# stephane-caron/pink

Measured on AMD Instinct MI355X. Metric: ik_qp_solves_per_s, higher is better.
Workload: dtype f64

## Files before the change

### pink_amd/csrc/ik_common.h

```cpp
#pragma once

#include <cmath>
#include <cstdint>
#include <type_traits>

#ifndef PINKHIP_GROUP_LARGE
#define PINKHIP_GROUP_LARGE 8
#endif
#ifndef PINKHIP_GROUP_SMALL
#define PINKHIP_GROUP_SMALL 4
#endif

#if defined(PINKHIP_TRACE) && !defined(__HIP_DEVICE_COMPILE__)
#include <cstdio>
#define PINKHIP_TRACEF(cond, ...)        \
  do {                                   \
    if (cond) std::printf(__VA_ARGS__);  \
  } while (0)
#else
#define PINKHIP_TRACEF(cond, ...)
#endif

namespace pinkhip {

template <int NV>
constexpr int group_size() {
  return NV >= 24 ? PINKHIP_GROUP_LARGE : PINKHIP_GROUP_SMALL;
}

template <int I, int N, class F>
__device__ __forceinline__ void static_for(F &&f) {
  if constexpr (I < N) {
    f(std::integral_constant<int, I>{});
    static_for<I + 1, N>(f);
  }
}
template <int W, int N, int BIT, class F>
__device__ __forceinline__ double transpose_reduce(F v) {
  const int lane = lane_id();
  if constexpr ((1 << BIT) >= W) {
    static_assert(N == 1, "N <= W values fold to one per lane");
    return v(std::integral_constant<int, 0>{});
  } else {
    constexpr int H = (N + 1) / 2;
    double nx[H];
    const bool up = ((lane >> BIT) & 1) != 0;
    static_for<0, H>([&](auto M) {
      constexpr int m = decltype(M)::value;
      const double a = v(std::integral_constant<int, 2 * m>{});
      double b = 0.0;
      if constexpr (2 * m + 1 < N) b = v(std::integral_constant<int, 2 * m + 1>{});
      nx[m] = (up ? b : a) + lane_shfl(up ? a : b, lane ^ (1 << BIT));
    });
    return transpose_reduce<W, H, BIT + 1>([&](auto K) { return nx[decltype(K)::value]; });
  }
}

typedef double TabVec16 __attribute__((vector_size(128)));
typedef double TabVec8 __attribute__((vector_size(64)));
template <bool HALF>
struct TabVecSel {
  typedef TabVec16 type;
};
template <>
struct TabVecSel<true> {
  typedef TabVec8 type;
};
template <int NT>
struct TabRegs {
  static constexpr int NVEC = (NT + 15) / 16;
  static_assert(NVEC >= 1 && NVEC <= 4, "at most 64 tableau columns");
  static constexpr bool kHalfLast = NT - 16 * (NVEC - 1) <= 8;
  template <int K>
  using Vec = typename TabVecSel<(K == NVEC - 1) && kHalfLast>::type;
  Vec<0> v0;
  Vec<1> v1;
  Vec<2> v2;
  Vec<3> v3;
  template <int K>
  __device__ __forceinline__ Vec<K> tuple() const {
    if constexpr (K == 0) return v0;
    else if constexpr (K == 1) return v1;
    else if constexpr (K == 2) return v2;
    else return v3;
  }
  template <int J>
  __device__ __forceinline__ double get() const {
    static_assert(J >= 0 && J < NT, "tableau column");
    const Vec<J / 16> t = tuple<J / 16>();
    return t[J % 16];
  }
  template <int J>
  __device__ __forceinline__ void set(double x) {
    static_assert(J >= 0 && J < NT, "tableau column");
    Vec<J / 16> t = tuple<J / 16>();
    t[J % 16] = x;
    if constexpr (J / 16 == 0) v0 = t;
    else if constexpr (J / 16 == 1) v1 = t;
    else if constexpr (J / 16 == 2) v2 = t;
    else v3 = t;
  }
  __device__ __forceinline__ void clear() {
    v0 = Vec<0>{};
    v1 = Vec<1>{};
    v2 = Vec<2>{};
    v3 = Vec<3>{};
  }
  __device__ __forceinline__ double at_uniform(int p) const {
    const int hi = p >> 4;
    const int lo = opaque_uniform(p & 15);
    const int lo8 = kHalfLast ? opaque_uniform(p & 7) : lo;
    const Vec<0> t0 = v0;
    double r = t0[NVEC == 1 ? lo8 : lo];
    if constexpr (NVEC > 1) {
      const Vec<1> t1 = v1;
      const double r1 = t1[NVEC == 2 ? lo8 : lo];
      r = (hi == 1) ? r1 : r;
    }
    if constexpr (NVEC > 2) {
      const Vec<2> t2 = v2;
      const double r2 = t2[NVEC == 3 ? lo8 : lo];
      r = (hi == 2) ? r2 : r;
    }
    if constexpr (NVEC > 3) {
      const Vec<3> t3 = v3;
      const double r3 = t3[lo8];
      r = (hi == 3) ? r3 : r;
    }
    return r;
  }
  template <int W>
  __device__ __forceinline__ double at_group_uniform(int p) const {
    constexpr int G = kWave / W;
    static_assert(G == 1 || G == 2, "one or two reads per wave");
    const int p0 = bcast_i(p, 0);
    double c = at_uniform(p0 < 0 ? 0 : p0);
    if constexpr (G == 2) {
      const int p1 = bcast_i(p, W);
      const double c1 = at_uniform(p1 < 0 ? 0 : p1);
      c = (lane_id() >= W) ? c1 : c;
    }
    return (p >= 0) ? c : 0.0;
  }
};

struct alignas(16) Pair {
  double a, b;
};

constexpr int STATUS_OPTIMAL = 0;
constexpr int STATUS_MAX_ITER = 1;
constexpr int STATUS_INFEASIBLE = 2;
constexpr int STATUS_NOT_PD = 3;
constexpr int STATUS_BREAKDOWN = 4;
constexpr int STATUS_ROUTED = 5;
constexpr int PATH_TABLEAU = 0, PATH_HANDOVER = 1, PATH_ROUTED = 2, PATH_GI = 3;
constexpr int kPathShift = 24;

struct KernelArgs {
  long long B;
  int nv, Kd, K, md;
  int n_eq;
  int n_dtasks;
  int n_barriers;
  int cost_batched;
  int max_iter;
  int lds_pitch;
  int rank_deficient;
  int n_free_lead;
  double damping, dt;
  double out_scale;
  const double *J, *e, *cost, *lb, *ub, *Gd, *hd, *c_extra;
  const double *row_gain;
  const double *row_lm;
  const int *dtask_col0;
  const int *dtask_row0;
  const int *dtask_k;
  const int *barrier_rows;
  const double *barrier_safe_gain;
  double *dq;
  int *status;
  int *iters;
  double *H_out, *c_out;
  const uint8_t *active_in;
  uint8_t *active_out;
};


}
// ... 1 lines not shown
```

### pink_amd/csrc/ik_stack_rows.h

```cpp
#pragma once

#include "ik_common.h"

namespace pinkhip {

struct HbmTerms {
  static constexpr bool kOnTheFly = false;
  double lb = 0.0, ub = 0.0, x = 0.0;
  int status = 0;
  __device__ __forceinline__ void frame_rows(int, double (&)[6]) const {}
  __device__ __forceinline__ double error(int) const { return 0.0; }
  __device__ __forceinline__ double diag_error(int) const { return 0.0; }
  __device__ __forceinline__ double dense_col(int) const { return 0.0; }
  __device__ __forceinline__ double dense_h(int) const { return 0.0; }
};

struct NoMid {
  __device__ __forceinline__ void operator()() const {}
};
template <int NX>
struct StackFront {
  double m[NX > 0 ? NX : 1] = {};
  double hxx[NX > 0 ? NX * (NX + 1) / 2 : 1] = {};
  double cx[NX > 0 ? NX : 1] = {};
};
template <int NV, int W, int RCMAX, class Src, int DEPTH = 1, int NX = 0, int NM, class Mid = NoMid>
__device__ __forceinline__ void stack_rows_bcast(const KernelArgs &a, long long b, Src *terms, bool in, int li,
                                                 double (&M)[NM], double &ci, double &mu_l, Mid mid = Mid(), StackFront<NX> *front = nullptr) {
  static_assert(NX >= 0 && NX <= 2 && (NX == 0 || !Src::kOnTheFly), "at most two front columns, from HBM");
  static_assert(NM >= NV && W >= 16, "row-group kernels only");
  using BcT = Bcast<W>;
  const int nv = a.nv, Kd = a.Kd, K = a.K;
  const double *Jb = a.J + b * (long long)Kd * nv;
  const double *eb = a.e + b * (long long)K;
  const double *costb = a.cost_batched ? a.cost + b * (long long)K : a.cost;
  constexpr int RC = Src::kOnTheFly ? 6 : (RCMAX < 8 ? RCMAX : 8);
  constexpr int NB = Src::kOnTheFly ? 2 : DEPTH + 1;
  static_assert(RC <= 16, "weight rows are broadcast from the first row of 16 lanes");
  struct Chunk {
    double r[RC];
    double pw, pe, pg, pl;
    double px[NX > 0 ? NX : 1];
  };
  Chunk buf[NB];
  auto request = [&](Chunk &dst, int r0) {
    const int rc = (Kd - r0 < RC) ? Kd - r0 : RC;
    if constexpr (Src::kOnTheFly) {
      double six[6];
      terms->frame_rows(r0 / 6, six);
#pragma unroll
      for (int kk = 0; kk < RC; ++kk) dst.r[kk] = (in && kk < rc) ? six[kk] : 0.0;
    } else {
#pragma unroll
      for (int kk = 0; kk < RC; ++kk) dst.r[kk] = (in && kk < rc) ? Jb[(long long)(r0 + kk) * nv + li] : 0.0;
    }
    dst.pw = dst.pe = dst.pg = dst.pl = 0.0;
    if constexpr (NX > 0) {
#pragma unroll
      for (int x = 0; x < NX; ++x) dst.px[x] = (li < rc) ? Jb[(long long)(r0 + li) * nv - NX + x] : 0.0;
    }
    if (li < rc) {
      const int k = r0 + li;
      dst.pw = costb[k];
      if constexpr (Src::kOnTheFly) dst.pe = terms->error(k);
      else dst.pe = eb[k];
      dst.pg = a.row_gain[k];
      dst.pl = a.row_lm[k];
    }
  };
  if (Kd > 0) {
#pragma unroll
    for (int d = 0; d < NB - 1; ++d)
      if (d * RC < Kd) request(buf[d], d * RC);
  }
  mid();
  for (int r0 = 0; r0 < Kd; r0 += RC) {
    const int rc = (Kd - r0 < RC) ? Kd - r0 : RC;
    if (r0 + (NB - 1) * RC < Kd) request(buf[NB - 1], r0 + (NB - 1) * RC);
    const Chunk &cur = buf[0];
    const double wa = (li < rc) ? cur.pw * cur.pw : 0.0;
    const double gw = (li < rc) ? cur.pg * wa * cur.pe : 0.0;
    if (li < rc) mu_l += cur.pl * (cur.pg * cur.pg) * wa * cur.pe * cur.pe;
    const BcT wab = bcast_prepare<W>(wa), gwb = bcast_prepare<W>(gw);
    BcT pxb[NX > 0 ? NX : 1];
    if constexpr (NX > 0) {
      front->hxx[0] = fma(wa * cur.px[0], cur.px[0], front->hxx[0]);
      front->cx[0] = fma(gw, cur.px[0], front->cx[0]);
      if constexpr (NX == 2) {
        front->hxx[1] = fma(wa * cur.px[0], cur.px[1], front->hxx[1]);
        front->hxx[2] = fma(wa * cur.px[1], cur.px[1], front->hxx[2]);
        front->cx[1] = fma(gw, cur.px[1], front->cx[1]);
      }
#pragma unroll
      for (int x = 0; x < NX; ++x) pxb[x] = bcast_prepare<W>(cur.px[x]);
    }
    static_for<0, RC>([&](auto Kc) {
      constexpr int kk = decltype(Kc)::value;
      if (kk < rc) {
        const double aa = fma_bcast<W, kk>(0.0, wab, cur.r[kk]);
        ci = fma_bcast<W, kk>(ci, gwb, cur.r[kk]);
        const BcT rowb = bcast_prepare<W>(cur.r[kk]);
        static_for<0, NV>([&](auto Jc) {
          constexpr int j = decltype(Jc)::value;
          M[j] = fma_bcast<W, j>(M[j], rowb, aa);
        });
        if constexpr (NX > 0) {
#pragma unroll
          for (int x = 0; x < NX; ++x) front->m[x] = fma_bcast<W, kk>(front->m[x], pxb[x], aa);
        }
      }
    });
#pragma unroll
    for (int d = 0; d + 1 < NB; ++d) buf[d] = buf[d + 1];
  }
}

template <class Src>
__device__ __forceinline__ double stack_diag_tasks(const KernelArgs &a, long long b, Src *terms, int li, double &ci,
                                                   double &mu_l) {
  const double *eb = a.e + b * (long long)a.K;
  const double *costb = a.cost_batched ? a.cost + b * (long long)a.K : a.cost;
  double dadd = 0.0;
  for (int t = 0; t < a.n_dtasks; ++t) {
    const int off = li - a.dtask_col0[t];
    if (off >= 0 && off < a.dtask_k[t]) {
      const int r = a.dtask_row0[t] + off;
      const double w = costb[r], gn = a.row_gain[r], l = a.row_lm[r];
      double ev;
      if constexpr (Src::kOnTheFly) ev = terms->diag_error(r);
      else ev = eb[r];
      const double wa = w * w;
      dadd += wa;
      ci += gn * wa * ev;
      mu_l += l * (gn * gn) * wa * ev * ev;
    }
  }
  return dadd;
}

}
```

### pink_amd/csrc/ik_sweep.h

```cpp
#pragma once

#include "ik_common.h"
#include "ik_kernels_packed.h"
#include "ik_stack_rows.h"

#ifdef PINKHIP_SECTION_CLOCK
#ifndef PINKHIP_TICK
static __device__ unsigned long long pinkhip_clock[16];
#define PINKHIP_TICK(k)                                                        \
  do {                                                                         \
    if (clock_on) {                                                            \
      const unsigned long long now_ = __builtin_readcyclecounter();            \
      if (lane == 0) atomicAdd(&pinkhip_clock[k], now_ - clock_prev);          \
      clock_prev = __builtin_readcyclecounter();                               \
    }                                                                          \
  } while (0)
#endif
#else
#ifndef PINKHIP_TICK
#define PINKHIP_TICK(k)
#endif
#endif

#ifndef PINKHIP_SWEEP_COLUMN_CHAINS
#define PINKHIP_SWEEP_COLUMN_CHAINS(NT) 2
#endif

#ifndef PINKHIP_SWEEP_CERT_TOL
#define PINKHIP_SWEEP_CERT_TOL 1e-12
#endif
#ifndef PINKHIP_STACK_DEPTH
#define PINKHIP_STACK_DEPTH 1
#endif
#ifndef PINKHIP_STACK_DEPTH_WIDE
#define PINKHIP_STACK_DEPTH_WIDE 2
#endif
#ifndef PINKHIP_SWEEP_INDEXED_COLUMN
#define PINKHIP_SWEEP_INDEXED_COLUMN 1
#endif
#ifndef PINKHIP_SWEEP_ROUTE_COND
#define PINKHIP_SWEEP_ROUTE_COND 1e8
#endif
#ifndef PINKHIP_SWEEP_PPM
#define PINKHIP_SWEEP_PPM 1
#endif
#ifndef PINKHIP_SWEEP_PPM_CRASH
#define PINKHIP_SWEEP_PPM_CRASH 1
#endif
#ifndef PINKHIP_ROLLOUT_PPM_DENSE
#define PINKHIP_ROLLOUT_PPM_DENSE 0
#endif
#ifndef PINKHIP_ROLLOUT_PPM_VIRTUAL
#define PINKHIP_ROLLOUT_PPM_VIRTUAL 0
#endif
#ifndef PINKHIP_SWEEP_PPM_DENSE
#define PINKHIP_SWEEP_PPM_DENSE 1
#endif
#ifdef PINKHIP_SWEEP_DEBUG_WHY
#define PINKHIP_WHY(k) why = (k) + 10 * status_before
#else
#define PINKHIP_WHY(k)
#endif
#ifndef PINKHIP_SWEEP_PPM_MIN_CURV
#define PINKHIP_SWEEP_PPM_MIN_CURV 1e-5
#endif
#ifndef PINKHIP_SWEEP_PPM_MURTY_AFTER
#define PINKHIP_SWEEP_PPM_MURTY_AFTER(nv) (4 * (nv) + 20)
#endif

namespace pinkhip {

template <int NV, int MD, int W>
struct SweepLds {
  static __host__ __device__ constexpr int tri(int i) { return i * (i + 1) / 2; }
  static constexpr int oC = (NV * (NV + 1) / 2 + 1) & ~1;
  static constexpr int GP = W + 2;
  static constexpr int oG = oC + W;
  static constexpr int oR = oG + MD * GP;
  static constexpr int stride = oR + W;
};

template <int NVT, int MD, int W, class Src = HbmTerms, bool WARM = false>
__device__ __forceinline__ int ik_sweep_instance(const KernelArgs &a, long long block, Src *terms = nullptr) {
  constexpr int NE = NVT > W ? NVT - W : 0;
  constexpr int NV = NVT - NE;
  static_assert(NE == 0 || (NE <= 2 && MD == 0 && !Src::kOnTheFly), "front coordinates are eliminated in the box-only stack + solve kernel");
  constexpr int NT = NV + MD;
  static_assert((W == 16 || W == 32 || W == 64) && NT <= W && NV % 2 == 0 && MD >= 0, "group of whole rows of 16 lanes");
  constexpr bool DENSE = MD > 0;
  constexpr bool PPM = !DENSE && PINKHIP_SWEEP_PPM;
  constexpr bool PPMD = DENSE && PINKHIP_SWEEP_PPM && PINKHIP_SWEEP_PPM_DENSE && (!Src::kOnTheFly || PINKHIP_ROLLOUT_PPM_DENSE);
  constexpr bool PPX = PPM || PPMD;
  static_assert(!WARM || PPM, "a warm start is a start of the principal pivoting of the box-only instantiations");
  constexpr int G = kWave / W;
  constexpr double INF = INFINITY;
  constexpr double BIG = 1e300;
  using BcT = Bcast<W>;

  const int lane = lane_id();
  const int g = lane / W, li = lane & (W - 1);
  const int nvs = a.nv;
  const int nv = nvs - NE;
  const int md = DENSE ? a.md : 0, n_eq = DENSE ? a.n_eq : 0;
#ifdef PINKHIP_SECTION_CLOCK
  const bool clock_on = (block & 63) == 0;
  unsigned long long clock_prev = __builtin_readcyclecounter();
#endif
  long long b = block * G + g;
  const bool valid = b < a.B;
  if (!valid) b = a.B - 1;

  const bool in = li < nv;
  const int dr = li - NV;
  const bool dlane = DENSE && dr >= 0 && dr < md;

  double T[NT];
#pragma unroll
  for (int j = 0; j < NT; ++j) T[j] = 0.0;
  double ci = 0.0, mu_l = 0.0, dadd = 0.0;
  double ci_d = 0.0, mu_d = 0.0, lbv = -INF, ubv = INF, hv = 0.0, ginv = 1.0;
  double front_dadd[NE > 0 ? NE : 1] = {}, front_c[NE > 0 ? NE : 1] = {};
  bool front_free = true;
  auto others = [&]() {
    if (in) {
      if constexpr (!Src::kOnTheFly) {
        lbv = a.lb[b * (long long)nvs + NE + li];
        ubv = a.ub[b * (long long)nvs + NE + li];
      }
      dadd = stack_diag_tasks<Src>(a, b, terms, NE + li, ci_d, mu_d);
      if (a.c_extra) ci_d += a.c_extra[b * (long long)nvs + NE + li];
    }
    if constexpr (NE > 0) {
#pragma unroll
      for (int x = 0; x < NE; ++x) {
        double mu_x = 0.0;
        front_dadd[x] = stack_diag_tasks<Src>(a, b, terms, x, front_c[x], mu_x);
        if (a.c_extra) front_c[x] += a.c_extra[b * (long long)nvs + x];
        if (li == x) mu_d += mu_x;
        front_free = front_free && a.lb[b * (long long)nvs + x] == -INF && a.ub[b * (long long)nvs + x] == INF;
      }
    }
    if constexpr (DENSE && !Src::kOnTheFly) {
      if (md > 0) {
        const double *Gb = a.Gd + b * (long long)md * nv;
        static_for<0, MD>([&](auto Dc) {
          constexpr int d = decltype(Dc)::value;
          T[NV + d] = (in && d < md) ? Gb[(long long)d * nv + li] : 0.0;
        });
        if (dlane) hv = a.hd[b * (long long)md + dr];
      }
    }
  };
  StackFront<NE> front;
  if constexpr (NE > 0) {
    KernelArgs af = a;
    af.J = a.J + NE;
    stack_rows_bcast<NV, W, 8, Src, PINKHIP_STACK_DEPTH, NE>(af, b, terms, in, li, T, ci, mu_l, others, &front);
  } else {
    stack_rows_bcast<NV, W, 8, Src, (NT > 34 ? PINKHIP_STACK_DEPTH_WIDE : PINKHIP_STACK_DEPTH)>(a, b, terms, in, li, T, ci, mu_l, others);
  }
  ci += ci_d;
  mu_l += mu_d;
  double diag = a.damping + group_sum<W>(mu_l);

  if constexpr (DENSE) {
    if (md > 0) {
      const double *Gb = Src::kOnTheFly ? nullptr : a.Gd + b * (long long)md * nv;
      if constexpr (Src::kOnTheFly) {
        static_for<0, MD>([&](auto Dc) {
          constexpr int d = decltype(Dc)::value;
          T[NV + d] = (in && d < md) ? terms->dense_col(d) : 0.0;
        });
      }
      if constexpr (Src::kOnTheFly) {
        static_for<0, MD>([&](auto Dc) {
          constexpr int d = decltype(Dc)::value;
          if (d < md) {
            const BcT gb = bcast_prepare<W>(T[NV + d]);
            static_for<0, NV>([&](auto Jc) {
              constexpr int j = decltype(Jc)::value;
              const double v = value_bcast<W, j>(gb);
              if (dr == d) T[j] = v;
            });
          }
        });
      }
      if (dlane) {
        double n2 = 0.0;
        if constexpr (!Src::kOnTheFly) {
          const double *gr = Gb + (long long)dr * nv;
#pragma unroll
          for (int j = 0; j < NV; ++j) T[j] = (j < nv) ? gr[j] : 0.0;
        } else {
          hv = terms->dense_h(dr);
        }
#pragma unroll
        for (int j = 0; j < NV; ++j) n2 += T[j] * T[j];
        ginv = (n2 > 0.0) ? 1.0 / sqrt(n2) : 1.0;
      }
      for (int t = 0; t < a.n_barriers; ++t) {
        const double r = a.barrier_safe_gain[t];
        if (r > 1e-6) {
          const int r0 = a.barrier_rows[t], r1 = a.barrier_rows[t + 1];
          double s = 0.0;
          static_for<0, MD>([&](auto Dc) {
            constexpr int d = decltype(Dc)::value;
            if (in && d >= r0 && d < r1) s += T[NV + d] * T[NV + d];
          });
          s = group_sum<W>(s);
          diag += r / (s * a.dt * a.dt);
        }
      }
    }
  }
  const double diag_u = diag;
  diag += dadd;
  double hii = 1.0;
#pragma unroll
  for (int j = 0; j < NV; ++j)
    if (j == li) {
      T[j] += in ? diag : 1.0;
      hii = T[j];
    }
  using SL = SweepLds<NV, MD, W>;
  double *sm = shared_base() + (long long)g * (a.lds_pitch ? a.lds_pitch : SL::stride);
  bool front_bad = false;
  if constexpr (NE > 0) {
    double h00 = group_sum<W>(front.hxx[0]) + diag_u + front_dadd[0];
    double c0 = group_sum<W>(front.cx[0]) + front_c[0];
    double h01 = 0.0, h11 = 1.0, c1 = 0.0;
    if constexpr (NE == 2) {
      h01 = group_sum<W>(front.hxx[1]);
      h11 = group_sum<W>(front.hxx[2]) + diag_u + front_dadd[1];
      c1 = group_sum<W>(front.cx[1]) + front_c[1];
    }
    const double m0 = in ? front.m[0] : 0.0;
    double m1 = (NE == 2 && in) ? front.m[NE - 1] : 0.0;
    front_bad = !(h00 > 0.0);
    const double r0 = fast_rcp(h00);
    {
      const BcT hb = bcast_prepare<W>(m0);
      const double f = -m0 * r0;
      static_for<0, NV>([&](auto Jc) {
        constexpr int j = decltype(Jc)::value;
        T[j] = fma_bcast<W, j>(T[j], hb, f);
      });
      ci = fma(f, c0, ci);
      hii = fma(f, m0, hii);
      if constexpr (NE == 2) {
        m1 = fma(f, h01, m1);
        h11 = fma(-h01 * r0, h01, h11);
        c1 = fma(-h01 * r0, c0, c1);
      }
    }
    double r1 = 0.0;
    if constexpr (NE == 2) {
      front_bad = front_bad || !(h11 > 0.0);
      r1 = fast_rcp(h11);
      const BcT hb = bcast_prepare<W>(m1);
      const double f = -m1 * r1;
      static_for<0, NV>([&](auto Jc) {
        constexpr int j = decltype(Jc)::value;
        T[j] = fma_bcast<W, j>(T[j], hb, f);
      });
      ci = fma(f, c1, ci);
      hii = fma(f, m1, hii);
    }
    wave_sync();
    sm[SL::stride + li] = m0;
    sm[SL::stride + W + li] = m1;
    if (li == 0) {
      double *fs = sm + SL::stride + 2 * W;
      fs[0] = c0, fs[1] = r0, fs[2] = h01, fs[3] = c1, fs[4] = r1;
    }
  }
  wave_sync();
  if (li < NV) {
#pragma unroll
    for (int j = 0; j < NV; ++j)
      if (j <= li) sm[SL::tri(li) + j] = T[j];
  }
  sm[SL::oC + li] = ci;
  if constexpr (DENSE) {
    static_for<0, MD>([&](auto Dc) {
      constexpr int d = decltype(Dc)::value;
      sm[SL::oG + d * SL::GP + li] = (li < NV) ? T[NV + d] : 0.0;
    });
  }
  PINKHIP_TICK(0);

  int status = STATUS_OPTIMAL;
  int why = 0, status_before = 0;
  if constexpr (NE > 0) {
    if (!front_free) status = STATUS_ROUTED;
    else if (front_bad) status = STATUS_NOT_PD;
  }
  double pmin = INF;
  int state = 0;
  if constexpr (Src::kOnTheFly) {
    lbv = in ? terms->lb : -INF;
    ubv = in ? terms->ub : INF;
  }
  constexpr bool GUESS = (PPX && PINKHIP_SWEEP_PPM_CRASH && !Src::kOnTheFly) || WARM;
  if constexpr (GUESS) {
    if (group_first_lane<W>(in && !(hii > 0.0)) < W) status = STATUS_NOT_PD;
    if constexpr (WARM) {
      const uint8_t *hint = a.active_in;
      if (hint) {
        if (in) {
          const int v = hint[b * (long long)nvs + NE + li];
          state = (v == 1 && lbv > -INF) ? 1 : ((v == 2 && ubv < INF) ? 2 : 0);
        }
      } else if constexpr (!Src::kOnTheFly) {
        const double xd = -ci * approx_rcp(hii);
        if (in) state = (xd < lbv) ? 1 : ((xd > ubv) ? 2 : 0);
      }
    } else {
      const double xd = -ci * approx_rcp(hii);
      if (in) state = (xd < lbv) ? 1 : ((xd > ubv) ? 2 : 0);
    }
    const unsigned long long fm = wave_ballot(li < NV && state == 0 && in);
    using FreeMask = typename std::conditional<W == 64, unsigned long long, unsigned>::type;
    FreeMask gfree = static_cast<FreeMask>(fm);
    if constexpr (W == 32) gfree = (lane >= 32) ? static_cast<unsigned>(fm >> 32) : static_cast<unsigned>(fm);
    else if constexpr (W == 16) gfree = static_cast<unsigned>(fm >> (lane & 48)) & 0xFFFFu;
    static_for<0, NV>([&](auto Kc) {
      constexpr int k = decltype(Kc)::value;
      {
        const bool want = ((gfree >> k) & 1) != 0;
        if (lanes_on(want)) {
          BcT xb = bcast_prepare<W>(T[k]);
          const double p = value_bcast<W, k>(xb);
          pmin = min_raw(pmin, want ? p : INF);
          const double rp = fast_rcp(p);
          const double t = T[k] * rp;
          double nt = (li == k) ? rp - 1.0 : -t;
          if (!want) nt = 0.0;
          double tk = (li == k) ? -rp : t;
#if defined(__HIP_DEVICE_COMPILE__)
          asm volatile("" : "+v"(nt), "+v"(xb.r[0]), "+v"(tk));
#endif
          static_for<0, NT>([&](auto Jc) {
            constexpr int j = decltype(Jc)::value;
            if constexpr (j != k) T[j] = fma_bcast<W, j>(T[j], xb, nt);
          });
          if (want) T[k] = tk;
        }
      }
    });
  }
  if constexpr (!GUESS) {
    static_for<0, NV>([&](auto Kc) {
      constexpr int k = decltype(Kc)::value;
      if (k < nv) {
        const BcT xb = bcast_prepare<W>(T[k]);
        const double p = value_bcast<W, k>(xb);
        pmin = min_raw(pmin, p);
        const double rp = fast_rcp(p);
        const double t = T[k] * rp;
        const double nt = (li == k) ? rp - 1.0 : -t;
        static_for<0, NT>([&](auto Jc) {
          constexpr int j = decltype(Jc)::value;
          if constexpr (j != k) T[j] = fma_bcast<W, j>(T[j], xb, nt);
        });
        T[k] = (li == k) ? -rp : t;
      }
    });
  }
  if (!(pmin > 0.0)) status = STATUS_NOT_PD;
  PINKHIP_TICK(1);
  double tdiag = 0.0;
#pragma unroll
  for (int j = 0; j < NT; ++j)
    if (j == li) tdiag = T[j];

  double x = 0.0, u = 0.0;
  {
    double vstart = in ? ci : 0.0;
    if constexpr (PPX) {
      if (state != 0) vstart = -((state == 1) ? lbv : ubv);
    }
    const BcT cb = bcast_prepare<W>(vstart);
    double r0 = 0.0, r1 = 0.0;
    static_for<0, NV>([&](auto Jc) {
      constexpr int j = decltype(Jc)::value;
      if constexpr (j % 2 == 0) r0 = fma_bcast<W, j>(r0, cb, T[j]);
      else r1 = fma_bcast<W, j>(r1, cb, T[j]);
    });
    x = in ? r0 + r1 : 0.0;
    if (dlane) u = hv + (r0 + r1);
    if constexpr (PPX) {
      if (state != 0) x -= ci;
    }
    if constexpr (PPMD) {
      if (dlane) x = u;
    }
  }
  double zd0 = -tdiag;
  if constexpr (PPMD) {
    const double hmax = -group_min<W>(in ? -hii : 0.0);
    zd0 = (li < NV) ? approx_rcp(hii) : approx_rcp(ginv * ginv * hmax);
  }
  {
    const double hii0 = (li < NV && in) ? sm[SL::tri(li < NV ? li : 0) + (li < NV ? li : 0)] : 0.0;
    const double kest = -group_min<W>((PPX && state != 0) ? -hii0 * approx_rcp(tdiag) : hii0 * tdiag);
    PINKHIP_TRACEF(li == 0, "[sweep g%d] kest %.3e\n", g, kest);
    if (status == STATUS_OPTIMAL && !(kest <= PINKHIP_SWEEP_ROUTE_COND)) status = STATUS_ROUTED;
  }
  PINKHIP_TICK(2);

  const KernelArgs *late = &a;
  if constexpr (!Src::kOnTheFly) late = kernarg_reload<KernelArgs>(a);
  const double tol = 1e-13 * (nv > 8 ? nv * 0.125 : 1.0);
  const double thr_lo = -tol * (1.0 + fabs(lbv)), thr_up = -tol * (1.0 + fabs(ubv));
  const double thr_d = -tol * (1.0 + fabs(hv) * ginv);
  const int max_iter = late->max_iter > 0 ? late->max_iter : 20 * (nv + md) + 50;
  const bool empty_box_somewhere = wave_any(in && ubv - lbv < (thr_lo > thr_up ? thr_lo : thr_up));
  double phi = 0.0, xfree = 1.0;
  int it = 0, eq_next = 0, src = 0, kind = 0;
  double uplus = 0.0;
  double blo = lbv, bhi = ubv, tlo = thr_lo, thi = thr_up;
  double thr_row = 0.0;
  if constexpr (PPMD) {
    thr_row = thr_d * fast_rcp(ginv);
    if (li >= NV) {
      blo = dlane ? 0.0 : -INF;
      bhi = INF;
      tlo = (dlane && dr >= n_eq) ? thr_row : -INF;
      thi = 0.0;
    }
  }
  if constexpr (PPX) {
    if (state != 0) {
      blo = (state == 1) ? -INF : 0.0;
      bhi = (state == 1) ? 0.0 : INF;
      tlo = 0.0;
      thi = 0.0;
    }
    if (empty_box_somewhere) {
      const bool empty = group_first_lane<W>(in && ubv - lbv < (thr_lo > thr_up ? thr_lo : thr_up)) < W;
      if (empty && status == STATUS_OPTIMAL) status = STATUS_INFEASIBLE;
    }
  }
  bool at_point = false;
  bool running = (status == STATUS_OPTIMAL);
  bool need_sel = true;
  bool refined = (status == STATUS_ROUTED);
  int nref = 0;
  double dprev = 0.0;

  auto krow_times = [&](double v) -> double {
    const BcT vb = bcast_prepare<W>(v);
    const int base = (li < NV) ? SL::tri(li) : SL::oG + (dlane ? dr : 0) * SL::GP;
    double h0 = 0.0, h1 = 0.0;
    static_for<0, NV>([&](auto Jc) {
      constexpr int j = decltype(Jc)::value;
      const int ad = (li < NV && j > li) ? SL::tri(j) + li : base + j;
      const double hv_ = sm[ad];
      if constexpr (j % 2 == 0) h0 = fma_bcast<W, j>(h0, vb, hv_);
      else h1 = fma_bcast<W, j>(h1, vb, hv_);
    });
    return h0 + h1;
  };
  auto residual = [&](bool &fails) -> double {
    const double kx = krow_times(in ? x : 0.0);
    const double ci_ = in ? sm[SL::oC + li] : 0.0;
    double grad = in ? kx + ci_ : 0.0;
    bool arow = false;
    if constexpr (DENSE) {
      if (md > 0) {
        arow = dlane && state == 1;
        const BcT lamb = bcast_prepare<W>(arow ? u : 0.0);
        double gl = 0.0;
        static_for<0, MD>([&](auto Dc) {
          constexpr int d = decltype(Dc)::value;
          gl = fma_bcast<W, NV + d>(gl, lamb, sm[SL::oG + d * SL::GP + li]);
        });
        if (in) grad += gl;
      }
    }
    const double hii = in ? sm[SL::tri(li < NV ? li : 0) + (li < NV ? li : 0)] : 0.0;
    const double gsc = group_min<W>(-hii) * group_min<W>(in ? -fabs(x) : 0.0) - group_min<W>(-fabs(ci_));
    const double gtol = PINKHIP_SWEEP_CERT_TOL * gsc;
    fails = false;
    if (in) {
      if (state == 0) fails = !(fabs(grad) <= gtol && x - lbv >= 10.0 * thr_lo && ubv - x >= 10.0 * thr_up);
      else fails = (state == 1) ? !(grad >= -gtol) : !(grad <= gtol);
    }
#if defined(PINKHIP_SWEEP_DEBUG_WHY) && defined(__HIP_DEVICE_COMPILE__)
    if (fails) printf("[cert blk %lld g%d li%d it%d nref%d] state %d x %.17g lb %.17g ub %.17g grad %.3e gtol %.3e thr %.3e %.3e\n", block, g, li, it, nref, state, x,
                      lbv, ubv, grad, gtol, thr_lo, thr_up);
#endif
    double r = (in && state == 0) ? grad : 0.0;
    if constexpr (DENSE) {
      if (dlane) {
        const double slack = (hv - kx) * ginv;
        if (arow) {
          r = kx - hv;
          fails = !(fabs(slack) <= -10.0 * thr_d) || (dr >= n_eq && !(u >= -gtol * ginv));
        } else if (state == 0 && dr >= n_eq) {
          fails = !(slack >= 10.0 * thr_d);
        }
      }
    }
    return r;
  };

#ifndef PINKHIP_SWEEP_LDS_COLUMN
#define PINKHIP_SWEEP_LDS_COLUMN 0
#endif
  double sdiag_run = tdiag;
  double *rowbuf = sm + SL::oR;
  constexpr bool IDX = PINKHIP_SWEEP_INDEXED_COLUMN && !PINKHIP_SWEEP_LDS_COLUMN && W >= 32;
  TabRegs<IDX ? NT : 1> R;
  R.clear();
  if constexpr (IDX) {
    static_for<0, NT>([&](auto Jc) {
      constexpr int j = decltype(Jc)::value;
      R.template set<j>(T[j]);
    });
  }
  auto tget = [&](auto Jc) -> double {
    constexpr int j = decltype(Jc)::value;
    if constexpr (IDX) return R.template get<j>();
    else return T[j];
  };
  auto tset = [&](auto Jc, double v) {
    constexpr int j = decltype(Jc)::value;
    if constexpr (IDX) R.template set<j>(v);
    else T[j] = v;
  };
  auto column_of = [&](int p) -> double {
    if constexpr (IDX) {
      return R.template at_group_uniform<W>(p);
    } else if constexpr (PINKHIP_SWEEP_LDS_COLUMN) {
      if (li == p) {
        Pair *dst = reinterpret_cast<Pair *>(__builtin_assume_aligned(rowbuf, 16));
#pragma unroll
        for (int j = 0; j + 1 < NT; j += 2) dst[j >> 1] = Pair{T[j], T[j + 1]};
        if constexpr (NT % 2) rowbuf[NT - 1] = T[NT - 1];
      }
      wave_sync();
      const double c = rowbuf[li < NT ? li : 0];
      wave_sync();
      return (p >= 0 && li < NT) ? c : 0.0;
    } else {
      const BcT eb = bcast_indicator<W>(p);
      constexpr int NC = PINKHIP_SWEEP_COLUMN_CHAINS(NT);
      double c[NC] = {};
      static_for<0, NT>([&](auto Jc) {
        constexpr int j = decltype(Jc)::value;
        c[j % NC] = fma_bcast<W, j>(c[j % NC], eb, tget(Jc));
      });
      if constexpr (NC == 4) return (c[0] + c[1]) + (c[2] + c[3]);
      else return c[0] + c[1];
    }
  };

  auto pivot_on = [&](int pi, double col, double pvt, double rp, double sg) {
    double t = col * rp;
    double cp = col;
    if (li == pi) {
      t = 1.0 - sg * rp;
      cp = pvt - sg;
    }
    const BcT xb = bcast_prepare<W>(cp);
    const double nt = -t;
    static_for<0, NT>([&](auto Jc) {
      constexpr int j = decltype(Jc)::value;
      tset(Jc, fma_bcast<W, j>(tget(Jc), xb, nt));
    });
    sdiag_run = fma(cp, nt, sdiag_run);
    tdiag = (li == pi) ? -rp : tdiag - t * col;
  };

  bool ppm_mode = PPX;
  bool restoring = false;
  const bool cand_lane = in || (DENSE && dlane && dr >= n_eq);
  const bool eq_lane = DENSE && dlane && dr < n_eq;

  for (;;) {
    double viol = 0.0;
    int nb_src = 0;
    bool iseq = false;
    if constexpr (PPX) {
      if (wave_any(running && ppm_mode)) {
        const bool sel = running && ppm_mode;
        const double slo = x - blo, sup = bhi - x;
        bool ok_lane = in, nonbasic = state != 0;
        if constexpr (DENSE) {
          nonbasic = (li < NV) ? (state != 0) : (state == 0);
          ok_lane = cand_lane && (!restoring || ((li < NV) ? (state != 0) : (state == 1)));
        }
        const bool vlo = ok_lane && slo < tlo, vup = ok_lane && sup < thi;
        viol = vlo ? slo : sup;
        if constexpr (DENSE) {
          if (eq_lane) viol = slo;
        }
        const float zf = fabsf(static_cast<float>(tdiag));
        const float wz = (zf > 1e-30f) ? approx_rcpf(zf) : 1e30f;
        const float fv = static_cast<float>(viol);
        float key = -(fv * fv) * wz;
        if (it > PINKHIP_SWEEP_PPM_MURTY_AFTER(nv + md)) key = static_cast<float>(li - 64);
        const float best32 = group_min32<W>((vlo || vup) ? key32_packf(key, li | (vlo ? 0 : 64) | (nonbasic ? 128 : 0)) : 3.0e38f);
        bool conv = false;
        if (sel) {
          if (DENSE && !restoring && eq_next < n_eq) {
            src = NV + eq_next;
            kind = 0;
            nb_src = 1;
            iseq = true;
// ... 205 lines not shown
              if (state != 0) {
                x = ((state == 1) ? lbv : ubv) + nu;
                state = 0;
                blo = lbv;
                bhi = ubv;
                tlo = thr_lo;
                thi = thr_up;
              } else {
                x = -nu;
                state = kind + 1;
                blo = kind ? 0.0 : -INF;
                bhi = kind ? INF : 0.0;
                tlo = 0.0;
                thi = 0.0;
              }
            } else if (state == 0) {
              x = nu;
              state = 1;
              tlo = 0.0;
              if (dr < n_eq) blo = -INF;
            } else {
              x = -nu;
              state = 0;
              tlo = thr_row;
            }
          }
          if constexpr (DENSE) {
            if (iseq) ++eq_next;
          }
        }
        PINKHIP_TICK(5);
        PINKHIP_TICK(6);
      }
    }
    if constexpr (!PPM) {
    if (!PPMD || wave_any(act && !ppm_mode)) {
    const bool actG = act && !ppm_mode;
    double cand = (kind == 0 ? lbv : ubv) - x;
    if constexpr (DENSE) cand = (li < NV) ? cand : -u;
    const double num = group_bcast<W>(cand, src);
    double pv = group_bcast<W>(tdiag, src);
    bool lin_dep = false;
    if constexpr (DENSE) {
      const double z0 = group_bcast<W>(zd0, src);
      const bool little = actG && !(-pv * 1e6 > z0);
      if (wave_any(little)) {
        const double w = (in && state == 0) ? col : 0.0;
        const double hw = krow_times(w);
        const double curv = group_sum<W>((li < NV) ? w * hw : 0.0);
        if (little) pv = -curv;
      }
      lin_dep = !(-pv * 1e12 > z0);
      PINKHIP_TRACEF(li == 0 && actG, "[sweep g%d it%d] enter src %d kind %d num %.3e pv %.3e z0 %.3e little %d lin_dep %d\n", g, it, src, kind,
                     num, pv, z0, (int)little, (int)lin_dep);
    }
    PINKHIP_TICK(4);
    const double rpv = fast_rcp(pv);
    const double sgn = (num >= 0.0) ? 1.0 : -1.0;
    const double full = lin_dep ? BIG : -fabs(num) * rpv;
    const double rate = phi * col * sgn;
    const bool blocking = actG && rate > 0.0;
    const double ratio = blocking ? max_raw(u, 0.0) * fast_rcp1(rate) : BIG;
    const double k1 = group_min<W>(ratio);
    const int kd = group_first_lane<W>(blocking && ratio == k1) & (W - 1);
    const double tstep = (k1 < full) ? k1 : full;
    const bool stuck = !(tstep < BIG);
    double hs = 0.0;
    if constexpr (DENSE) {
      if (wave_any(actG && stuck)) hs = group_bcast<W>((li < NV) ? (kind == 0 ? lbv : ubv) : hv, src);
    }
    if (actG && stuck) {
      const bool tiny = DENSE && fabs(num) <= 1e-9 * (1.0 + fabs(hs));
      PINKHIP_TRACEF(li == 0, "[sweep g%d it%d] stuck: src %d kind %d num %.3e hs %.3e pv %.3e lin_dep %d k1 %.3e full %.3e tiny %d\n",
                     g, it, src, kind, num, hs, pv, (int)lin_dep, k1, full, (int)tiny);
      if (kind == 3 && tiny) {
        ++eq_next;
        need_sel = true;
      } else if (tiny) {
        if (li == src) {
          if (li >= NV) hv -= u, u = 0.0;
          else if (kind == 0) lbv = x;
          else ubv = x;
        }
        need_sel = true;
      } else {
        status = STATUS_INFEASIBLE;
        running = false;
      }
    }
    const bool act2 = actG && running && !stuck;
    const bool do_add = act2 && !(k1 < full);
    const bool do_drop = act2 && !do_add;
    {
      const double nu = act2 ? sgn * tstep : 0.0;
      const double d = col * nu;
      x = fma(-xfree, d, x);
      u = fma((DENSE && li >= NV) ? -1.0 : -phi, d, u);
      if constexpr (DENSE) uplus += (kind == 3) ? nu : fabs(nu);
      else uplus += fabs(nu);
    }
    PINKHIP_TICK(5);
    if (do_add) {
      pi = src;
      pvt = pv;
      rp = rpv;
      if (li == src) {
        if (li < NV) {
          state = kind + 1;
          x = (kind == 0) ? lbv : ubv;
          phi = (kind == 0) ? -1.0 : 1.0;
        } else {
          state = 1;
          phi = (DENSE && dr >= n_eq) ? 1.0 : 0.0;
        }
        xfree = 0.0;
        u = uplus;
      }
      if (DENSE && kind == 3) ++eq_next;
      need_sel = true;
    }
    if (wave_any(do_drop)) {
      const double ck = column_of(do_drop ? kd : -1);
      const double pk = group_bcast<W>(tdiag, kd);
      if (do_drop) {
        col = (li == kd) ? tdiag : ck;
        pi = kd;
        pvt = pk;
        rp = fast_rcp(pk);
        if (li == kd) {
          state = 0;
          u = 0.0;
          phi = 0.0;
          xfree = 1.0;
        }
      }
    }
    PINKHIP_TICK(6);
    if (!ppm_mode) sg = ((!DENSE || pi < NV) == do_add) ? -1.0 : 1.0;
    }
    }
    pivot_on(pi, col, pvt, rp, sg);
    PINKHIP_TICK(7);
  }
  PINKHIP_TICK(8);
  if constexpr (Src::kOnTheFly) {
    terms->x = in ? x : 0.0;
    terms->status = status;
  }
  {
    int ln = lane;
#if defined(__HIP_DEVICE_COMPILE__)
    asm volatile("" : "+v"(ln));
#endif
    const long long bw = block * G + ln / W;
    double xe[NE > 0 ? NE : 1] = {};
    if constexpr (NE > 0) {
      const double *fs = sm + SL::stride + 2 * W;
      const double xr = in ? x : 0.0;
      if constexpr (NE == 2) xe[1] = -(fs[3] + group_sum<W>(sm[SL::stride + W + li] * xr)) * fs[4];
      xe[0] = -(fs[0] + group_sum<W>(sm[SL::stride + li] * xr) + ((NE == 2) ? fs[2] * xe[NE - 1] : 0.0)) * fs[1];
    }
    if (bw < late->B) {
      if (in) late->dq[bw * (long long)nvs + NE + li] = x * late->out_scale;
      if constexpr (NE > 0) {
        if (li < NE) late->dq[bw * (long long)nvs + li] = ((li == 0) ? xe[0] : xe[NE - 1]) * late->out_scale;
      }
      if (li == 0) {
        late->status[bw] = status;
        if (late->iters) late->iters[bw] = it + 1000 * why;
      }
      if constexpr (WARM) {
        uint8_t *const aout = late->active_out;
        if (aout) {
          if (in) aout[bw * (long long)nvs + NE + li] = static_cast<uint8_t>(status == STATUS_OPTIMAL ? state : 0);
          if constexpr (NE > 0) {
            if (li < NE) aout[bw * (long long)nvs + li] = 0;
          }
        }
      }
    }
  }
  PINKHIP_TRACEF(li == 0, "[sweep g%d] exit status %d it %d nref %d\n", g, status, it, nref);
  return status;
}

template <int NV, int MD, int W>
__host__ __device__ constexpr int sweep_kernel_lds_doubles(int md) {
  return SweepLds<NV, MD, W>::stride > LdsP<NV>::stride(MD > 0 ? md : 0) ? SweepLds<NV, MD, W>::stride : LdsP<NV>::stride(MD > 0 ? md : 0);
}

template <int NV, int MD, int W, bool WARM = false>
__device__ __forceinline__ void ik_solve_sweep_body(const KernelArgs &a, long long block) {
  const int st = ik_sweep_instance<NV, MD, W, HbmTerms, WARM>(a, block);
#ifndef PINKHIP_SWEEP_NO_HANDOVER
#ifdef PINKHIP_SWEEP_FORCE_HANDOVER
  const bool over = true;
#else
  const bool over = st == STATUS_BREAKDOWN || st == STATUS_ROUTED;
#endif
  if (wave_any(over)) {
    wave_sync();
    const KernelArgs *again = kernarg_reload<KernelArgs>(a);
    long long blk = block;
#if defined(__HIP_DEVICE_COMPILE__)
    asm volatile("" : "+s"(blk));
#endif
    if constexpr (NV > W) {
      constexpr int G = kWave / W;
      const int path = st == STATUS_ROUTED ? PATH_ROUTED : PATH_HANDOVER;
      static_for<0, G>([&](auto Gc) {
        constexpr int gg = decltype(Gc)::value;
        const bool og = bcast_i(over ? 1 : 0, gg * W) != 0;
        const int pg = bcast_i(path, gg * W);
        if (og && blk * G + gg < again->B) {
          wave_sync();
          ik_packed_instance<NV, kWave, false, HbmTerms, WARM>(*again, blk * G + gg, static_cast<HbmTerms *>(nullptr), true, pg);
        }
      });
    } else {
      ik_packed_instance<NV, W, (MD > 0), HbmTerms, WARM>(*again, blk, static_cast<HbmTerms *>(nullptr), over, st == STATUS_ROUTED ? PATH_ROUTED : PATH_HANDOVER);
    }
  }
#endif
}

template <int NV, int MD, int W>
__global__ void __launch_bounds__(kWave) PINKHIP_OCCUPANCY_SWEEP3(NV, MD, W) ik_solve_sweep_kernel(KernelArgs a) {
  ik_solve_sweep_body<NV, MD, W>(a, block_id());
}

template <int NV, int MD, int W>
__global__ void __launch_bounds__(kWave) PINKHIP_OCCUPANCY_SWEEP3(NV, MD, W) ik_solve_sweep_warm_kernel(KernelArgs a) {
  ik_solve_sweep_body<NV, MD, W, true>(a, block_id());
}

}
```

Baseline: 181.2 million.

## Use wave-uniform base pointers and track tableau diagonal in registers

```diff
diff --git a/pink_amd/csrc/ik_common.h b/pink_amd/csrc/ik_common.h
--- a/pink_amd/csrc/ik_common.h
+++ b/pink_amd/csrc/ik_common.h
@@ -35,6 +35,26 @@
     static_for<I + 1, N>(f);
   }
 }
+template <int W, int J>
+__device__ __forceinline__ double add_in_lane(double t, double d) {
+  static_assert((W == 16 || W == 32 || W == 64) && J >= 0 && J < W, "lane of a group of whole rows of 16 lanes");
+#if defined(__HIP_DEVICE_COMPILE__)
+  constexpr unsigned long long one = 1ull << J;
+  constexpr unsigned long long m = W == 64 ? one : W == 32 ? one | (one << 32) : one | (one << 16) | (one << 32) | (one << 48);
+  unsigned slo, shi;
+  asm("s_mov_b32 %1, exec_lo\n\ts_mov_b32 %2, exec_hi\n\t"
+      "s_and_b32 exec_lo, %1, %4\n\ts_and_b32 exec_hi, %2, %5\n\t"
+      "v_add_f64 %0, %0, %3\n\t"
+      "s_mov_b32 exec_lo, %1\n\ts_mov_b32 exec_hi, %2"
+      : "+v"(t), "=&s"(slo), "=&s"(shi)
+      : "v"(d), "n"(static_cast<int>(m & 0xFFFFFFFFull)), "n"(static_cast<int>(m >> 32))
+      : "scc");
+  return t;
+#else
+  return ((lane_id() & (W - 1)) == J) ? t + d : t;
+#endif
+}
+
 template <int W, int N, int BIT, class F>
 __device__ __forceinline__ double transpose_reduce(F v) {
   const int lane = lane_id();
diff --git a/pink_amd/csrc/ik_stack_rows.h b/pink_amd/csrc/ik_stack_rows.h
--- a/pink_amd/csrc/ik_stack_rows.h
+++ b/pink_amd/csrc/ik_stack_rows.h
@@ -24,16 +24,28 @@
   double hxx[NX > 0 ? NX * (NX + 1) / 2 : 1] = {};
   double cx[NX > 0 ? NX : 1] = {};
 };
-template <int NV, int W, int RCMAX, class Src, int DEPTH = 1, int NX = 0, int NM, class Mid = NoMid>
+struct WaveSplit {
+  long long first = 0;
+  unsigned rel = 0;
+};
+#ifndef PINKHIP_WAVE_SPLIT
+#define PINKHIP_WAVE_SPLIT(Src) (!Src::kOnTheFly)
+#endif
+template <int NV, int W, int RCMAX, class Src, int DEPTH = 1, int NX = 0, bool DIAG = false, int NM, class Mid = NoMid>
 __device__ __forceinline__ void stack_rows_bcast(const KernelArgs &a, long long b, Src *terms, bool in, int li,
-                                                 double (&M)[NM], double &ci, double &mu_l, Mid mid = Mid(), StackFront<NX> *front = nullptr) {
+                                                 double (&M)[NM], double &ci, double &mu_l, Mid mid = Mid(), StackFront<NX> *front = nullptr,
+                                                 double *hdiag = nullptr, WaveSplit ws = WaveSplit()) {
   static_assert(NX >= 0 && NX <= 2 && (NX == 0 || !Src::kOnTheFly), "at most two front columns, from HBM");
   static_assert(NM >= NV && W >= 16, "row-group kernels only");
   using BcT = Bcast<W>;
   const int nv = a.nv, Kd = a.Kd, K = a.K;
-  const double *Jb = a.J + b * (long long)Kd * nv;
-  const double *eb = a.e + b * (long long)K;
-  const double *costb = a.cost_batched ? a.cost + b * (long long)K : a.cost;
+  constexpr bool SPLIT = DIAG && PINKHIP_WAVE_SPLIT(Src);
+  const double *Jb = a.J + (SPLIT ? ws.first : b) * (long long)Kd * nv;
+  const double *eb = a.e + (SPLIT ? ws.first : b) * (long long)K;
+  const double *costb = a.cost_batched ? a.cost + (SPLIT ? ws.first : b) * (long long)K : a.cost;
+  const unsigned voJ = SPLIT ? ws.rel * static_cast<unsigned>(Kd * nv) + li : 0u;
+  const unsigned voE = SPLIT ? ws.rel * static_cast<unsigned>(K) + li : 0u;
+  const unsigned voC = (SPLIT && a.cost_batched) ? voE : static_cast<unsigned>(li);
   constexpr int RC = Src::kOnTheFly ? 6 : (RCMAX < 8 ? RCMAX : 8);
   constexpr int NB = Src::kOnTheFly ? 2 : DEPTH + 1;
   static_assert(RC <= 16, "weight rows are broadcast from the first row of 16 lanes");
@@ -52,20 +64,34 @@
       for (int kk = 0; kk < RC; ++kk) dst.r[kk] = (in && kk < rc) ? six[kk] : 0.0;
     } else {
 #pragma unroll
-      for (int kk = 0; kk < RC; ++kk) dst.r[kk] = (in && kk < rc) ? Jb[(long long)(r0 + kk) * nv + li] : 0.0;
+      for (int kk = 0; kk < RC; ++kk) {
+        if constexpr (SPLIT) dst.r[kk] = (in && kk < rc) ? (Jb + (long long)(r0 + kk) * nv)[voJ] : 0.0;
+        else dst.r[kk] = (in && kk < rc) ? Jb[(long long)(r0 + kk) * nv + li] : 0.0;
+      }
     }
     dst.pw = dst.pe = dst.pg = dst.pl = 0.0;
     if constexpr (NX > 0) {
 #pragma unroll
-      for (int x = 0; x < NX; ++x) dst.px[x] = (li < rc) ? Jb[(long long)(r0 + li) * nv - NX + x] : 0.0;
+      for (int x = 0; x < NX; ++x) {
+        if constexpr (SPLIT) dst.px[x] = (li < rc) ? (Jb + ((long long)r0 * nv - NX + x))[voJ - li + static_cast<unsigned>(li * nv)] : 0.0;
+        else dst.px[x] = (li < rc) ? Jb[(long long)(r0 + li) * nv - NX + x] : 0.0;
+      }
     }
     if (li < rc) {
       const int k = r0 + li;
-      dst.pw = costb[k];
-      if constexpr (Src::kOnTheFly) dst.pe = terms->error(k);
-      else dst.pe = eb[k];
-      dst.pg = a.row_gain[k];
-      dst.pl = a.row_lm[k];
+      if constexpr (SPLIT) {
+        dst.pw = (costb + r0)[voC];
+        if constexpr (Src::kOnTheFly) dst.pe = terms->error(k);
+        else dst.pe = (eb + r0)[voE];
+        dst.pg = (a.row_gain + r0)[static_cast<unsigned>(li)];
+        dst.pl = (a.row_lm + r0)[static_cast<unsigned>(li)];
+      } else {
+        dst.pw = costb[k];
+        if constexpr (Src::kOnTheFly) dst.pe = terms->error(k);
+        else dst.pe = eb[k];
+        dst.pg = a.row_gain[k];
+        dst.pl = a.row_lm[k];
+      }
     }
   };
   if (Kd > 0) {
@@ -99,6 +125,7 @@
       if (kk < rc) {
         const double aa = fma_bcast<W, kk>(0.0, wab, cur.r[kk]);
         ci = fma_bcast<W, kk>(ci, gwb, cur.r[kk]);
+        if constexpr (DIAG) *hdiag = fma(cur.r[kk], aa, *hdiag);
         const BcT rowb = bcast_prepare<W>(cur.r[kk]);
         static_for<0, NV>([&](auto Jc) {
           constexpr int j = decltype(Jc)::value;
@@ -138,4 +165,29 @@
   return dadd;
 }
 
+template <class Src>
+__device__ __forceinline__ double stack_diag_tasks(const KernelArgs &a, WaveSplit ws, Src *terms, int li, double &ci,
+                                                   double &mu_l) {
+  const double *eb = a.e + ws.first * (long long)a.K;
+  const double *costb = a.cost_batched ? a.cost + ws.first * (long long)a.K : a.cost;
+  const unsigned vo = ws.rel * static_cast<unsigned>(a.K);
+  const unsigned voc = a.cost_batched ? vo : 0u;
+  double dadd = 0.0;
+  for (int t = 0; t < a.n_dtasks; ++t) {
+    const int off = li - a.dtask_col0[t];
+    if (off >= 0 && off < a.dtask_k[t]) {
+      const int r = a.dtask_row0[t] + off;
+      const double w = costb[voc + static_cast<unsigned>(r)], gn = a.row_gain[r], l = a.row_lm[r];
+      double ev;
+      if constexpr (Src::kOnTheFly) ev = terms->diag_error(r);
+      else ev = eb[vo + static_cast<unsigned>(r)];
+      const double wa = w * w;
+      dadd += wa;
+      ci += gn * wa * ev;
+      mu_l += l * (gn * gn) * wa * ev * ev;
+    }
+  }
+  return dadd;
 }
+
+}
diff --git a/pink_amd/csrc/ik_sweep.h b/pink_amd/csrc/ik_sweep.h
--- a/pink_amd/csrc/ik_sweep.h
+++ b/pink_amd/csrc/ik_sweep.h
@@ -68,6 +68,13 @@
 #define PINKHIP_SWEEP_PPM_MURTY_AFTER(nv) (4 * (nv) + 20)
 #endif
 
+#ifndef PINKHIP_SWEEP_DIAG_REGISTER
+#define PINKHIP_SWEEP_DIAG_REGISTER(Src) (!Src::kOnTheFly)
+#endif
+#ifndef PINKHIP_SWEEP_LATE_ADDRESSES
+#define PINKHIP_SWEEP_LATE_ADDRESSES(Src) (!Src::kOnTheFly)
+#endif
+
 namespace pinkhip {
 
 template <int NV, int MD, int W>
@@ -88,6 +95,7 @@
   constexpr int NT = NV + MD;
   static_assert((W == 16 || W == 32 || W == 64) && NT <= W && NV % 2 == 0 && MD >= 0, "group of whole rows of 16 lanes");
   constexpr bool DENSE = MD > 0;
+  constexpr bool DREG = PINKHIP_SWEEP_DIAG_REGISTER(Src);
   constexpr bool PPM = !DENSE && PINKHIP_SWEEP_PPM;
   constexpr bool PPMD = DENSE && PINKHIP_SWEEP_PPM && PINKHIP_SWEEP_PPM_DENSE && (!Src::kOnTheFly || PINKHIP_ROLLOUT_PPM_DENSE);
   constexpr bool PPX = PPM || PPMD;
@@ -109,6 +117,10 @@
   long long b = block * G + g;
   const bool valid = b < a.B;
   if (!valid) b = a.B - 1;
+  WaveSplit ws;
+  ws.first = (block * G < a.B - 1) ? block * G : a.B - 1;
+  ws.rel = static_cast<unsigned>(b - ws.first);
+  const unsigned vo = ws.rel * static_cast<unsigned>(nvs) + li;
 
   const bool in = li < nv;
   const int dr = li - NV;
@@ -124,11 +136,16 @@
   auto others = [&]() {
     if (in) {
       if constexpr (!Src::kOnTheFly) {
-        lbv = a.lb[b * (long long)nvs + NE + li];
-        ubv = a.ub[b * (long long)nvs + NE + li];
-      }
-      dadd = stack_diag_tasks<Src>(a, b, terms, NE + li, ci_d, mu_d);
-      if (a.c_extra) ci_d += a.c_extra[b * (long long)nvs + NE + li];
+        lbv = (a.lb + (ws.first * (long long)nvs + NE))[vo];
+        ubv = (a.ub + (ws.first * (long long)nvs + NE))[vo];
+      }
+      if constexpr (PINKHIP_WAVE_SPLIT(Src)) dadd = stack_diag_tasks<Src>(a, ws, terms, NE + li, ci_d, mu_d);
+      else dadd = stack_diag_tasks<Src>(a, b, terms, NE + li, ci_d, mu_d);
+      if constexpr (PINKHIP_WAVE_SPLIT(Src)) {
+        if (a.c_extra) ci_d += (a.c_extra + (ws.first * (long long)nvs + NE))[vo];
+      } else {
+        if (a.c_extra) ci_d += a.c_extra[b * (long long)nvs + NE + li];
+      }
     }
     if constexpr (NE > 0) {
 #pragma unroll
@@ -152,12 +169,13 @@
     }
   };
   StackFront<NE> front;
+  double hii = 0.0;
   if constexpr (NE > 0) {
     KernelArgs af = a;
     af.J = a.J + NE;
-    stack_rows_bcast<NV, W, 8, Src, PINKHIP_STACK_DEPTH, NE>(af, b, terms, in, li, T, ci, mu_l, others, &front);
+    stack_rows_bcast<NV, W, 8, Src, PINKHIP_STACK_DEPTH, NE, DREG>(af, b, terms, in, li, T, ci, mu_l, others, &front, &hii, ws);
   } else {
-    stack_rows_bcast<NV, W, 8, Src, (NT > 34 ? PINKHIP_STACK_DEPTH_WIDE : PINKHIP_STACK_DEPTH)>(a, b, terms, in, li, T, ci, mu_l, others);
+    stack_rows_bcast<NV, W, 8, Src, (NT > 34 ? PINKHIP_STACK_DEPTH_WIDE : PINKHIP_STACK_DEPTH), 0, DREG>(a, b, terms, in, li, T, ci, mu_l, others, nullptr, &hii, ws);
   }
   ci += ci_d;
   mu_l += mu_d;
@@ -215,13 +233,22 @@
   }
   const double diag_u = diag;
   diag += dadd;
-  double hii = 1.0;
+  if constexpr (DREG) {
+    const double dd = in ? diag : 1.0;
+    static_for<0, NV>([&](auto Jc) {
+      constexpr int j = decltype(Jc)::value;
+      T[j] = add_in_lane<W, j>(T[j], dd);
+    });
+    hii += dd;
+  } else {
+    hii = 1.0;
 #pragma unroll
-  for (int j = 0; j < NV; ++j)
-    if (j == li) {
-      T[j] += in ? diag : 1.0;
-      hii = T[j];
-    }
+    for (int j = 0; j < NV; ++j)
+      if (j == li) {
+        T[j] += in ? diag : 1.0;
+        hii = T[j];
+      }
+  }
   using SL = SweepLds<NV, MD, W>;
   double *sm = shared_base() + (long long)g * (a.lds_pitch ? a.lds_pitch : SL::stride);
   bool front_bad = false;
@@ -302,6 +329,7 @@
     ubv = in ? terms->ub : INF;
   }
   constexpr bool GUESS = (PPX && PINKHIP_SWEEP_PPM_CRASH && !Src::kOnTheFly) || WARM;
+  double tdiag = (li < NV) ? hii : 0.0;
   if constexpr (GUESS) {
     if (group_first_lane<W>(in && !(hii > 0.0)) < W) status = STATUS_NOT_PD;
     if constexpr (WARM) {
@@ -333,6 +361,8 @@
           const double p = value_bcast<W, k>(xb);
           pmin = min_raw(pmin, want ? p : INF);
           const double rp = fast_rcp(p);
+          double own = T[k];
+          if constexpr (DREG) opaque(own);
           const double t = T[k] * rp;
           double nt = (li == k) ? rp - 1.0 : -t;
           if (!want) nt = 0.0;
@@ -340,11 +370,14 @@
 #if defined(__HIP_DEVICE_COMPILE__)
           asm volatile("" : "+v"(nt), "+v"(xb.r[0]), "+v"(tk));
 #endif
+          double td = 0.0;
+          if constexpr (DREG) td = fma(own, nt, tdiag);
           static_for<0, NT>([&](auto Jc) {
             constexpr int j = decltype(Jc)::value;
             if constexpr (j != k) T[j] = fma_bcast<W, j>(T[j], xb, nt);
           });
           if (want) T[k] = tk;
+          if constexpr (DREG) tdiag = (li == k) ? T[k] : td;
         }
       }
     });
@@ -363,16 +396,21 @@
           constexpr int j = decltype(Jc)::value;
           if constexpr (j != k) T[j] = fma_bcast<W, j>(T[j], xb, nt);
         });
+        if constexpr (DREG) tdiag = (li == k) ? -rp : fma(T[k], nt, tdiag);
         T[k] = (li == k) ? -rp : t;
       }
     });
   }
   if (!(pmin > 0.0)) status = STATUS_NOT_PD;
   PINKHIP_TICK(1);
-  double tdiag = 0.0;
+  if constexpr (DREG) {
+    if (li >= NT) tdiag = 0.0;
+  } else {
+    tdiag = 0.0;
 #pragma unroll
-  for (int j = 0; j < NT; ++j)
-    if (j == li) tdiag = T[j];
+    for (int j = 0; j < NT; ++j)
+      if (j == li) tdiag = T[j];
+  }
 
   double x = 0.0, u = 0.0;
   {
@@ -451,12 +489,23 @@
 
   auto krow_times = [&](double v) -> double {
     const BcT vb = bcast_prepare<W>(v);
-    const int base = (li < NV) ? SL::tri(li) : SL::oG + (dlane ? dr : 0) * SL::GP;
+    constexpr bool LATE = PINKHIP_SWEEP_LATE_ADDRESSES(Src);
+    int lo_ = li;
+#if defined(__HIP_DEVICE_COMPILE__)
+    if constexpr (LATE) asm volatile("" : "+v"(lo_));
+#endif
+    const int base = (lo_ < NV) ? SL::tri(lo_) : SL::oG + (dlane ? dr : 0) * SL::GP;
+    const double *const rowp = sm + base, *const colp = sm + lo_;
     double h0 = 0.0, h1 = 0.0;
     static_for<0, NV>([&](auto Jc) {
       constexpr int j = decltype(Jc)::value;
-      const int ad = (li < NV && j > li) ? SL::tri(j) + li : base + j;
-      const double hv_ = sm[ad];
+      double hv_;
+      if constexpr (LATE) {
+        const double *const pj = (j > lo_) ? colp : rowp + (j - SL::tri(j));
+        hv_ = pj[SL::tri(j)];
+      } else {
+        hv_ = sm[(li < NV && j > li) ? SL::tri(j) + li : base + j];
+      }
       if constexpr (j % 2 == 0) h0 = fma_bcast<W, j>(h0, vb, hv_);
       else h1 = fma_bcast<W, j>(h1, vb, hv_);
     });
@@ -968,7 +1017,10 @@
 #if defined(__HIP_DEVICE_COMPILE__)
     asm volatile("" : "+v"(ln));
 #endif
-    const long long bw = block * G + ln / W;
+    const long long bw0 = block * G;
+    const unsigned gw = static_cast<unsigned>(ln) / W;
+    const long long bw = bw0 + gw;
+    const unsigned vow = gw * static_cast<unsigned>(nvs) + li;
     double xe[NE > 0 ? NE : 1] = {};
     if constexpr (NE > 0) {
       const double *fs = sm + SL::stride + 2 * W;
@@ -977,13 +1029,21 @@
       xe[0] = -(fs[0] + group_sum<W>(sm[SL::stride + li] * xr) + ((NE == 2) ? fs[2] * xe[NE - 1] : 0.0)) * fs[1];
     }
     if (bw < late->B) {
-      if (in) late->dq[bw * (long long)nvs + NE + li] = x * late->out_scale;
-      if constexpr (NE > 0) {
-        if (li < NE) late->dq[bw * (long long)nvs + li] = ((li == 0) ? xe[0] : xe[NE - 1]) * late->out_scale;
-      }
-      if (li == 0) {
-        late->status[bw] = status;
-        if (late->iters) late->iters[bw] = it + 1000 * why;
+      if constexpr (PINKHIP_WAVE_SPLIT(Src)) {
+        if (in) (late->dq + (bw0 * (long long)nvs + NE))[vow] = x * late->out_scale;
+        if constexpr (NE > 0) {
+          if (li < NE) (late->dq + bw0 * (long long)nvs)[vow] = ((li == 0) ? xe[0] : xe[NE - 1]) * late->out_scale;
+        }
+        if (li == 0) {
+          (late->status + bw0)[gw] = status;
+          if (late->iters) (late->iters + bw0)[gw] = it + 1000 * why;
+        }
+      } else {
+        if (in) late->dq[bw * (long long)nvs + NE + li] = x * late->out_scale;
+        if (li == 0) {
+          late->status[bw] = status;
+          if (late->iters) late->iters[bw] = it + 1000 * why;
+        }
       }
       if constexpr (WARM) {
         uint8_t *const aout = late->active_out;
```

Result: faster. 185.0 million, median of 6 (+2.1%).
